# kakaoenterprise/JORLDY

Measured on AMD Instinct MI355X. Metric: env_steps_per_s (PPO CartPole sync, W=8 workers/GPU, T=128), higher is better.
Workload: dtype f32

## Files before the change

include/jorldy_hip.h:

```cpp
#ifndef JORLDY_HIP_H
#define JORLDY_HIP_H

#include <stdint.h>

#ifdef __cplusplus
extern "C" {
#endif

#define JH_ABI_VERSION 2

typedef enum {
  JH_OK = 0,
  JH_ERR_HIP = -1,
  JH_ERR_ARG = -2,
  JH_ERR_STATE = -3,
  JH_ERR_NOMEM = -4,
  JH_ERR_NODEVICE = -5
} jh_status;

typedef enum { JH_U8 = 0, JH_F32 = 1, JH_I64 = 2, JH_F64 = 3, JH_I32 = 4 } jh_dtype;

typedef struct jh_ctx jh_ctx;
typedef struct jh_store jh_store;
typedef struct jh_per jh_per;
// ... 37 lines not shown
void* jh_store_col_ptr(jh_store* s, int32_t col);
int64_t jh_store_size(const jh_store* s);
int64_t jh_store_index(const jh_store* s);
int64_t jh_store_capacity(const jh_store* s);
void jh_store_clear(jh_store* s);
int jh_store_set_position(jh_store* s, int64_t index, int64_t counter);

int jh_per_create(jh_ctx* ctx, int64_t capacity, double uniform_sample_prob, jh_per** out);
void jh_per_destroy(jh_per* p);
int jh_per_push(jh_per* p, int64_t n, const double* h_prio, jh_stream stream);
int jh_per_push_device(jh_per* p, int64_t n, const double* d_prio, jh_stream stream);
int jh_per_update(jh_per* p, int64_t B, const int64_t* d_idx, const void* d_prio, int32_t prio_dtype, jh_stream stream);
int jh_per_sample(jh_per* p, int64_t B, double beta, int64_t n_uniform, const int64_t* h_uniform_slot,
                  const double* h_u, int64_t* d_idx, double* d_w64, float* d_w32, double* d_stats, jh_stream stream);
int jh_per_shard_stats(jh_per* p, int64_t B, double* d_out3, jh_stream stream);
int jh_per_weights_sharded(jh_per* p, int64_t B, double beta, const double* d_all3, int32_t n_shards, double* d_w64,
                           float* d_w32, jh_stream stream);
int jh_per_state(jh_per* p, double* max_priority, double* root, int64_t* tree_index, int64_t* counter, jh_stream stream);
double* jh_per_tree_ptr(jh_per* p);
int64_t jh_per_tree_size(const jh_per* p);
int jh_per_load(jh_per* p, const double* h_tree, double max_priority, int64_t tree_index, int64_t counter);
int jh_per_dump(jh_per* p, double* h_tree, jh_stream stream);

int jh_gae(jh_ctx* ctx, int32_t W, int32_t T, float gamma, float lambda, const float* d_reward, const float* d_done,
           const float* d_value, const float* d_next_value, float* d_adv, float* d_ret, int32_t standardize,
           jh_stream stream);
int jh_ppo_minibatch_rows(jh_ctx* ctx, int64_t n, const int64_t* d_idx, int32_t n_cols, const int32_t* elems,
                          const float* const* d_src, float* const* d_dst, jh_stream stream);
int jh_mean_f32(jh_ctx* ctx, int64_t n, const float* d_x, float* d_out, jh_stream stream);
int jh_logp_discrete(jh_ctx* ctx, int64_t M, int32_t A, const float* d_logits, const float* d_action, float* d_logp,
                     jh_stream stream);
int jh_logp_continuous(jh_ctx* ctx, int64_t M, int32_t A, const float* d_mu_raw, const float* d_log_std_raw,
                       const float* d_action, float* d_logp, jh_stream stream);
int jh_ppo_loss_discrete(jh_ctx* ctx, int32_t B, int32_t A, const float* d_logits, const float* d_value_pred,
                         const int64_t* d_idx, const float* d_action, const float* d_adv, const float* d_ret,
                         const float* d_value_old, const float* d_logp_old, float eps_clip, float vf_coef,
                         float ent_coef, float* d_grad_logits, float* d_grad_value, float* d_stats,
                         jh_stream stream);
int jh_ppo_loss_continuous(jh_ctx* ctx, int32_t B, int32_t A, const float* d_mu_raw, const float* d_log_std_raw,
                           const float* d_value_pred, const int64_t* d_idx, const float* d_action, const float* d_adv,
                           const float* d_ret, const float* d_value_old, const float* d_logp_old, float eps_clip,
                           float vf_coef, float ent_coef, float* d_grad_mu_raw, float* d_grad_log_std_raw,
                           float* d_grad_value, float* d_stats, jh_stream stream);
int jh_ppo_loss_deferred(jh_ctx* ctx, int32_t continuous, int32_t B, int32_t A, const float* d_head0, const float* d_head1,
                         const float* d_value_pred, const int64_t* d_idx, const float* d_action, const float* d_adv, const float* d_ret,
                         const float* d_value_old, const float* d_logp_old, float eps_clip, float vf_coef, float ent_coef,
                         float* d_grad_head0, float* d_grad_head1, float* d_grad_value, float* d_dv2, float* d_critic_sums,
                         float* d_stats_local, jh_stream stream);
int jh_ppo_critic_select_rows(jh_ctx* ctx, int32_t B, const float* d_critic_sums, float vf_coef, float ent_coef, float* d_grad_value,
                              const float* d_dv2, const float* d_stats_local, float* d_stats, jh_stream stream);

int jh_ppo_loss_packed(jh_ctx* ctx, int32_t continuous, int32_t B, int32_t A, const float* d_heads, int32_t ld, const int64_t* d_idx, const float* d_action,
                       const float* d_adv, const float* d_ret, const float* d_value_old, const float* d_logp_old, float eps_clip, float vf_coef,
                       float ent_coef, float* d_grad_heads, float* d_dv2, float* d_critic_sums, float* d_stats, jh_stream stream);
int jh_ppo_critic_select_strided(jh_ctx* ctx, int32_t B, const float* d_critic_sums, float vf_coef, float ent_coef, float* d_grad_value, int32_t ldv,
                                 const float* d_dv2, const float* d_stats_local, float* d_stats, jh_stream stream);
int jh_heads_unpack(jh_ctx* ctx, int64_t rows, int32_t A, const float* d_packed, int32_t ld, float* d_h0, float* d_h1, float* d_value, jh_stream stream);
int jh_policy_act_discrete(jh_ctx* ctx, int32_t W, int32_t A, const float* d_heads, int32_t ld, uint64_t seed, uint64_t counter, int32_t training,
                           int64_t* d_action, jh_stream stream);

#define JH_TD_DOUBLE 1
#define JH_TD_PER 2
int jh_td_loss(jh_ctx* ctx, int32_t B, int32_t A, int32_t n_step, int32_t flags, const float* d_q,
               const float* d_q_next_online, const float* d_q_next_target, const float* d_action,
               const float* d_reward, const float* d_done, const float* d_weights, float gamma, float alpha,
               float* d_grad_q, float* d_prio, float* d_stats, jh_stream stream);
// ... 327 lines not shown
```

jorldy_amd/_lib.py:

```python
import ctypes as C
import os

_HERE = os.path.dirname(os.path.abspath(__file__))
LIB_PATH = os.path.join(_HERE, "csrc", "libjorldy_hip.so")

JH_U8, JH_F32, JH_I64, JH_F64, JH_I32 = 0, 1, 2, 3, 4
JH_TD_DOUBLE, JH_TD_PER = 1, 2
JH_C51_DOUBLE, JH_C51_PER, JH_C51_SHIFT_MAX = 1, 2, 4


class JhError(RuntimeError):
    pass


class ColDesc(C.Structure):
    _fields_ = [("dtype", C.c_int32), ("elems", C.c_int64)]


_vp, _i32, _i64, _f32, _f64 = C.c_void_p, C.c_int32, C.c_int64, C.c_float, C.c_double
_pp = C.POINTER(C.c_void_p)

_PROTOS = {
    "jh_abi_version": (C.c_int, []),
    "jh_stream_abort_capture": (C.c_int, [_vp]),
# ... 14 lines not shown
    "jh_pinned_free": (None, [_vp]),
    "jh_store_create": (C.c_int, [_vp, _i64, _i32, C.POINTER(ColDesc), _pp]),
    "jh_store_destroy": (None, [_vp]),
    "jh_store_push": (C.c_int, [_vp, _i64, _pp, _vp]),
    "jh_store_push_device": (C.c_int, [_vp, _i64, _pp, _vp]),
    "jh_store_stage_begin": (C.c_int, [_vp, _i64, _pp]),
    "jh_store_stage_commit": (C.c_int, [_vp, _vp]),
    "jh_store_write_rows": (C.c_int, [_vp, _i64, _vp, _pp, _vp]),
    "jh_store_gather": (C.c_int, [_vp, _i64, _vp, _i64, _i32, C.POINTER(_i32), _pp, C.POINTER(_i32), _vp]),
    "jh_store_col_ptr": (_vp, [_vp, _i32]),
    "jh_store_size": (_i64, [_vp]),
    "jh_store_index": (_i64, [_vp]),
    "jh_store_capacity": (_i64, [_vp]),
    "jh_store_clear": (None, [_vp]),
    "jh_store_set_position": (C.c_int, [_vp, _i64, _i64]),
    "jh_per_create": (C.c_int, [_vp, _i64, _f64, _pp]),
    "jh_per_destroy": (None, [_vp]),
    "jh_per_push": (C.c_int, [_vp, _i64, _vp, _vp]),
    "jh_per_push_device": (C.c_int, [_vp, _i64, _vp, _vp]),
    "jh_per_update": (C.c_int, [_vp, _i64, _vp, _vp, _i32, _vp]),
    "jh_per_sample": (C.c_int, [_vp, _i64, _f64, _i64, _vp, _vp, _vp, _vp, _vp, _vp, _vp]),
    "jh_per_state": (C.c_int, [_vp, C.POINTER(_f64), C.POINTER(_f64), C.POINTER(_i64), C.POINTER(_i64), _vp]),
    "jh_per_tree_ptr": (_vp, [_vp]),
    "jh_per_shard_stats": (C.c_int, [_vp, _i64, _vp, _vp]),
    "jh_per_weights_sharded": (C.c_int, [_vp, _i64, _f64, _vp, _i32, _vp, _vp, _vp]),
    "jh_per_tree_size": (_i64, [_vp]),
    "jh_per_load": (C.c_int, [_vp, _vp, _f64, _i64, _i64]),
    "jh_per_dump": (C.c_int, [_vp, _vp, _vp]),
    "jh_gae": (C.c_int, [_vp, _i32, _i32, _f32, _f32, _vp, _vp, _vp, _vp, _vp, _vp, _i32, _vp]),
    "jh_ppo_minibatch_rows": (C.c_int, [_vp, _i64, _vp, _i32, _vp, _vp, _vp, _vp]),
    "jh_mean_f32": (C.c_int, [_vp, _i64, _vp, _vp, _vp]),
    "jh_logp_discrete": (C.c_int, [_vp, _i64, _i32, _vp, _vp, _vp, _vp]),
    "jh_logp_continuous": (C.c_int, [_vp, _i64, _i32, _vp, _vp, _vp, _vp, _vp]),
    "jh_ppo_loss_discrete": (C.c_int, [_vp, _i32, _i32, _vp, _vp, _vp, _vp, _vp, _vp, _vp, _vp, _f32, _f32, _f32, _vp, _vp, _vp, _vp]),
    "jh_ppo_loss_continuous": (C.c_int, [_vp, _i32, _i32, _vp, _vp, _vp, _vp, _vp, _vp, _vp, _vp, _vp, _f32, _f32, _f32, _vp, _vp, _vp, _vp, _vp]),
    "jh_normal_fill": (C.c_int, [_vp, _i64, _vp, _vp, _vp]),
    "jh_value_act": (C.c_int, [_vp, _i32, _i32, _i32, _vp, _f32, _f32, _vp, _vp, _vp, _vp, _vp, _vp, _vp]),
    "jh_td_loss": (C.c_int, [_vp, _i32, _i32, _i32, _i32, _vp, _vp, _vp, _vp, _vp, _vp, _vp, _f32, _f32, _vp, _vp, _vp, _vp]),
    "jh_c51_loss": (C.c_int, [_vp, _i32, _i32, _i32, _i32, _i32, _vp, _vp, _vp, _vp, _vp, _vp, _vp, _f32, _f32, _f32, _f32, _vp, _vp, _vp, _vp, _vp]),
    "jh_mdqn_loss": (C.c_int, [_vp, _i32, _i32, _vp, _vp, _vp, _vp, _vp, _vp, _f32, _f32, _f32, _f32, _vp, _vp, _vp]),
    "jh_qr_loss": (C.c_int, [_vp, _i32, _i32, _i32, _vp, _vp, _vp, _vp, _vp, _vp, _vp, _f32, _vp, _vp, _vp]),
    "jh_quantile_act": (C.c_int, [_vp, _i32, _i32, _i32, _vp, _vp, _vp, _vp, _vp, _vp, _vp, _vp]),
    "jh_iqnnet_param_count_for": (_i64, [_i32, _i32, _i32, _i32, _i32]),
    "jh_iqnnet_create": (C.c_int, [_vp, _i32, _i32, _i32, _i32, _i32, _i32, _vp, _vp, _vp, _vp, _vp, _pp]),
    "jh_iqnnet_destroy": (None, [_vp]),
    "jh_iqnnet_segment_count": (_i32, []),
    "jh_iqnnet_segment": (C.c_int, [_vp, _i32, C.POINTER(_i64), C.POINTER(_i32), C.POINTER(_i32)]),
    "jh_iqnnet_set_hyper": (C.c_int, [_vp, _f64, _f64, _f64, _f64, _i64, _vp]),
    "jh_iqnnet_set_lr": (C.c_int, [_vp, _f64, _vp]),
    "jh_iqnnet_sync_target": (C.c_int, [_vp, _vp]),
    "jh_iqnnet_forward": (C.c_int, [_vp, _i32, _vp, _i32, _vp, _vp, _vp]),
    "jh_iqnnet_learn_forward": (C.c_int, [_vp, _vp, _i32, _vp, _vp, _vp]),
    "jh_iqnnet_learn_forward_m": (C.c_int, [_vp, _vp, _i32, _vp, _vp, _vp]),
    "jh_iqnnet_backward": (C.c_int, [_vp, _vp, _vp]),
    "jh_iqnnet_optim_step": (C.c_int, [_vp, _f32, _vp]),
    "jh_iqn_cos_features": (C.c_int, [_vp, _i64, _i32, _vp, _vp, _vp]),
    "jh_iqn_hadamard": (C.c_int, [_vp, _i32, _i32, _i32, _vp, _vp, _vp, _vp]),
    "jh_iqn_hadamard_backward": (C.c_int, [_vp, _i32, _i32, _i32, _vp, _vp, _vp, _vp, _vp, _vp]),
    "jh_iqn_loss": (C.c_int, [_vp, _i32, _i32, _i32, _vp, _vp, _vp, _vp, _vp, _vp, _vp, _f32, _vp, _vp, _vp]),
    "jh_miqn_loss": (C.c_int, [_vp, _i32, _i32, _i32, _vp, _vp, _vp, _vp, _vp, _vp, _vp, _f32, _f32, _f32, _f32, _vp, _vp, _vp]),
    "jh_iqn_act": (C.c_int, [_vp, _i32, _i32, _i32, _vp, _vp, _vp, _vp, _vp, _vp, _vp, _vp]),
    "jh_td3_next_action": (C.c_int, [_vp, _i32, _i32, _vp, _vp, _f32, _f32, _vp, _vp]),
    "jh_td3_critic_loss": (C.c_int, [_vp, _i32, _i32, _vp, _vp, _vp, _vp, _f32, _vp, _vp, _vp, _vp]),
    "jh_td3_actor_seed": (C.c_int, [_vp, _i32, _vp, _vp, _vp, _vp]),
    "jh_td3_tanh_backward": (C.c_int, [_vp, _i32, _i32, _vp, _vp, _vp, _vp]),
    "jh_td3_polyak": (C.c_int, [_vp, _i64, _vp, _vp, _f64, _vp]),
# ... 220 lines not shown
```

jorldy_amd/core/agent/ppo.py:

```python
import os

import numpy as np
import torch

from ... import np_rng, ops
from ..buffer import RolloutBuffer
from ..network import Network
from ..optimizer import Optimizer
from .base import BaseAgent


MAX_HEAD_OUTPUTS = 40
NATIVE_ELIGIBLE = ("PPO runs on libjorldy_hip only: network in {discrete_policy_value, continuous_policy_value}, head='mlp', int state_size, "
                   "hidden_size % 16 == 0, optim_config name 'adam' without weight_decay / amsgrad, and action_size + 1 (discrete) or "
                   f"2 * action_size + 1 (continuous) <= {MAX_HEAD_OUTPUTS} head outputs (config.ppo.cartpole, config.ppo.mujoco on all its envs; up to 8 outputs "
                   "-- CartPole, Hopper -- on the four-launch minibatch update and the persistent acting kernel, beyond that on the separate calls / the tiled engine); "
                   "head='cnn' with a (C, H, W) state_size and network 'discrete_policy_value' runs on the convolutional engine (core/agent/ppo_cnn.py: config.ppo.atari, ppo.procgen)")


class PPO(BaseAgent):

    def __new__(cls, *args, **kwargs):
        if cls is PPO and kwargs.get("head", args[4] if len(args) > 4 else "mlp") == "cnn":
            from .ppo_cnn import PPOConv

            return object.__new__(PPOConv)
        return object.__new__(cls)

    def __init__(self, state_size, action_size, hidden_size=512, network="discrete_policy_value", head="mlp",
                 optim_config={"name": "adam"}, gamma=0.99, use_standardization=True, run_step=1e6, lr_decay=True,
                 device=None, batch_size=32, n_step=128, n_epoch=3, _lambda=0.95, epsilon_clip=0.1, vf_coef=1.0,
                 ent_coef=0.01, clip_grad_norm=1.0, num_workers=1, backend=None, use_graph=True, seed=0, **kwargs):
        self.device = self._require_gpu(device)
        self.action_type = network.split("_")[0]
        assert self.action_type in ["continuous", "discrete"]
        if backend not in (None, "auto", "native"):
            raise ValueError(f"backend={backend!r}: jorldy_amd has one backend (libjorldy_hip); the torch mirror of round 1-3 is test infrastructure now (tests/mirror)")
        shape_ok = (head == "mlp" and isinstance(state_size, (int, np.integer)) and network in ("discrete_policy_value", "continuous_policy_value")
                    and hidden_size % 16 == 0 and optim_config.get("name", "adam").lower() == "adam"
                    and (2 * action_size + 1 if self.action_type == "continuous" else action_size + 1) <= MAX_HEAD_OUTPUTS)
        if not shape_ok:
            raise ValueError(f"{NATIVE_ELIGIBLE}; got network={network!r}, head={head!r}, state_size={state_size!r}, hidden_size={hidden_size}, "
                             f"optim_config={optim_config!r}, action_size={action_size}")
        self.network = Network(network, state_size, action_size, D_hidden=hidden_size, head=head).to(self.device)
        self.optimizer = Optimizer(**optim_config, params=self.network.parameters())
        self.gamma = gamma
        self.use_standardization = use_standardization
        self.memory = RolloutBuffer(device=self.device)
        self.run_step = run_step
        self.lr_decay = lr_decay
        self.batch_size = batch_size
        self.n_step = n_step
        self.n_epoch = n_epoch
# ... 2 lines not shown
        self.vf_coef = vf_coef
        self.ent_coef = ent_coef
        self.clip_grad_norm = clip_grad_norm
        self.num_workers = num_workers
        self.time_t = 0
        self.learn_stamp = 0
        self._stats = None
        self.grad_sync = None
        self.dp_exact_critic = os.environ.get("JH_DP_EXACT_CRITIC", "1") == "1"

        eligible = (
            head == "mlp" and isinstance(state_size, (int, np.integer)) and optim_config.get("name", "adam").lower() == "adam"
            and network in ("discrete_policy_value", "continuous_policy_value") and hidden_size % 16 == 0
            and not self.optimizer.defaults.get("amsgrad", False) and self.optimizer.defaults.get("weight_decay", 0) == 0
            and (2 * action_size + 1 if self.action_type == "continuous" else action_size + 1) <= MAX_HEAD_OUTPUTS
        )
        if not eligible:
            raise ValueError(f"{NATIVE_ELIGIBLE}; got network={network!r}, head={head!r}, state_size={state_size!r}, hidden_size={hidden_size}, "
                             f"optim_config={optim_config!r}, action_size={action_size}")
        self.backend = "native"
        self.use_graph = use_graph
        self.fused_update = os.environ.get("JH_FUSED_UPDATE", "1") == "1"
        self.graph_with_collective = os.environ.get("JH_GRAPH_DP", "1") == "1"
        self._net = None
        self._learn_graphs = ops.LearnGraphs("learn()")
        self._static = None
        self._adam_steps = 0
        self._captured = 0
        self._post_launch_hook = None
        self._lr_step = None
        self._ride, self._ride_done, self._ride_wait = None, False, {}
        self._lr_word = None
        self._predraw = np_rng.Predraw() if os.environ.get("JH_PPO_PREDRAW", "1") == "1" else None
        self._init_native(int(state_size), int(action_size), int(hidden_size), seed)

    def _init_native(self, S, A, H, seed, max_rows=4096):
        cont = self.action_type == "continuous"
        self._seed = seed
        net = ops.PPONet(S, H, A, cont, max_rows, self.device, seed=seed)
        params = list(self.network.parameters())
        assert sum(p.numel() for p in params) == net.n_params, "state_dict layout mismatch with libjorldy_hip"
        o = 0
        with torch.no_grad():
            for p in params:
                n = p.numel()
                net.params[o : o + n].copy_(p.reshape(-1))
                p.data = net.params[o : o + n].view_as(p)
                p.grad = net.grads[o : o + n].view_as(p)
                o += n
        self._views = [(p, net.m[a : a + p.numel()].view_as(p), net.v[a : a + p.numel()].view_as(p))
                       for p, a in zip(params, np.cumsum([0] + [q.numel() for q in params[:-1]]))]
        d = self.optimizer.defaults
        net.set_hyper(d["lr"], d["betas"][0], d["betas"][1], d["eps"], step=0.0)
        self._net = net

    def _grow_native(self, rows):
        if rows <= self._net.max_rows:
            return
        old = self._net
        S, H, A = old.S, old.H, old.A
        net = ops.PPONet(S, H, A, old.cont, max(rows, 2 * old.max_rows), self.device, seed=self._seed)
        for dst, src in ((net.params, old.params), (net.grads, old.grads), (net.m, old.m), (net.v, old.v)):
            dst.copy_(src)
        o = 0
        for p in self.network.parameters():
            n = p.numel()
# ... 75 lines not shown
            self._static = self._alloc_static(M)
            self.reset_graphs()
        st = self._static
        return st["h0"], st["h1"], st["value"], st["next_value"]

    def _drop_rides(self):
        if self._ride is not None:
            self._ride.clear_rides()
        self._ride_wait.clear()
        if self._static is not None:
            self._static["idx_ready"] = False

    def _upload_idx(self, st, draw, ride=False):
        k = st["idx_k"]
        st["idx_k"] = 1 - k
        if st["idx_ev"][k] is not None:
            st["idx_ev"][k].synchronize()
            st["idx_ev"][k] = None
        ok = draw(st["idx_pin"][k].np)
        if ok is False:
            return False
        if ride and self._ride is not None:
            self._ride.ride_along(0, st["idx_pin"][k].dev_ptr.value, st["idx"].data_ptr(), st["idx"].numel() * 8, keep=(st["idx_pin"][k], st["idx"]))
            self._ride_wait["idx"] = k
            return True
        self._ride_wait.pop("idx", None)
        st["idx"].copy_(st["idx_alias"][k])
        ev = torch.cuda.Event()
        ev.record()
        st["idx_ev"][k] = ev
        return True

    def _enqueue_learn(self, st, captured=False):
        self._enqueue_pre(st, captured)
        self._enqueue_main(st)

    def _enqueue_pre(self, st, captured=False):
        self._enqueue_gather(st)
        self._enqueue_pre_pass(st, captured)

    def _enqueue_gather(self, st):
        tr = st["tr"]
        self.memory._store.gather(st["arange"], as_float=True, out={k: tr[k] for k in tr})

    def _enqueue_pre_pass(self, st, captured=False):
        net, M = self._net, st["M"]
        cont = net.cont
        tr = st["tr"]
        if captured:
            pass
        elif 2 * M <= min(net.max_rows, 8192):
            net.forward(st["x_all"], out=(st["h0_all"], st["h1_all"], st["v_all"]))
        else:
            net.forward(tr["next_state"], out=(st["nh0"], st["nh1"], st["next_value"]))
            net.forward(tr["state"], out=(st["h0"], st["h1"], st["value"]))
        if cont:
            logp_old = ops.logp_continuous(st["h0"], st["h1"], tr["action"], out=st["logp_old"])
        else:
            logp_old = ops.logp_discrete(st["h0"], tr["action"], out=st["logp_old"])
        adv, ret = ops.gae(tr["reward"], tr["done"], st["value"], st["next_value"], self.n_step, self.gamma, self._lambda, self.use_standardization,
                           out=(st["adv"], st["ret"]))
        ops.mean_into(ret, st["stats"][st["n_upd"], 0:1])

    def _enqueue_main(self, st):
        net, M, B = self._net, st["M"], self.batch_size
        cont = net.cont
        tr, adv, ret, logp_old = st["tr"], st["adv"], st["ret"], st["logp_old"]
        k = 0
        if "rows" in st:
            xs, acts, advs, rets, vals, lps = st["rows"](st["idx"])
            exact = self.grad_sync is not None and self.dp_exact_critic
            if exact and "critic_sums" not in st:
                st["critic_sums"] = torch.zeros(st["n_upd"], 2, dtype=torch.float32, device=self.device)
            for e in range(self.n_epoch):
                for offset in range(0, M, B):
                    o0, o1 = e * M + offset, e * M + min(offset + B, M)
                    if exact:
                        net.ppo_update_dp(xs[o0:o1], None, acts[o0:o1], advs[o0:o1], rets[o0:o1], vals[o0:o1], lps[o0:o1], self.epsilon_clip, self.vf_coef,
                                          self.ent_coef, st["stats"][k], self.grad_sync.reduce_flat, st["critic_sums"][k],
                                          peer=getattr(getattr(self.grad_sync, "transport", None), "peer", None))
                    else:
                        net.ppo_update(xs[o0:o1], None, acts[o0:o1], advs[o0:o1], rets[o0:o1], vals[o0:o1], lps[o0:o1], self.epsilon_clip, self.vf_coef,
                                       self.ent_coef, self.clip_grad_norm, st["stats"][k], do_adam=self.grad_sync is None)
                    if self.grad_sync is not None:
                        self.grad_sync.reduce_flat(net.grads)
                        net.adam_step(self.clip_grad_norm)
                    k += 1
            return
        exact = self.grad_sync is not None and self.dp_exact_critic
        if exact and "dp_work" not in st:
            st["dp_work"] = torch.zeros(st["n_upd"], B + 16, dtype=torch.float32, device=self.device)
        onepass = not exact and os.environ.get("JH_PPO_ONEPASS", "1") == "1"
        for e in range(self.n_epoch):
            for offset in range(0, M, B):
                b = min(B, M - offset)
                idx = st["idx"][e * M + offset : e * M + offset + b]
                if onepass:
                    net.ppo_update_rows(tr["state"], idx, tr["action"], adv, ret, st["value"], logp_old, self.epsilon_clip, self.vf_coef, self.ent_coef, self.clip_grad_norm,
                                        st["stats"][k], do_adam=self.grad_sync is None)
                    if self.grad_sync is not None:
                        self.grad_sync.reduce_flat(net.grads)
                        net.adam_step(self.clip_grad_norm)
                    k += 1
# ... 45 lines not shown
        self._captured = 0
        rode, self._ride_done = self._ride_done, False
        if self._ride_wait and not rode:
            if "lr" in self._ride_wait:
                self._net.set_lr(float(self._lr_word.np[0]))
            if "idx" in self._ride_wait and st["idx_ready"]:
                st["idx"].copy_(st["idx_alias"][self._ride_wait["idx"]])
        self._ride_wait.clear()

        def shuffles():
            self._upload_idx(st, lambda out: np_rng.epoch_shuffles(M, E, out))

        pin = st.get("stats_pin")
        if pin is not None:
            pin.np[st["n_upd"] - 1, 2] = -1.0
            pin.np[st["n_upd"] - 1, 7] = -1.0
        graphable = (self.use_graph and not ops._PROF["on"]
                     and (self.grad_sync is None or (self.graph_with_collective and getattr(self.grad_sync, "capturable", True))))
        have_idx = bool(st["idx_ready"]) and self._predraw is not None and self._predraw.commit(M, E)
        st["idx_ready"] = False
        split = not have_idx and os.environ.get("JH_PPO_SPLIT_GRAPH", "1") == "1"
        key = ("split" if split else "one", captured)
        lg, pre = self._learn_graphs, lambda: self._enqueue_pre(st, captured)
        bodies = {key: pre, "main": lambda: self._enqueue_main(st)} if split else {key: lambda: self._enqueue_learn(st, captured)}
        if lg.ready(key, bodies, graphable, warm_key=key, capture=allow_capture):
            if split:
                lg.replay(key)
                shuffles()
                lg.replay("main")
            else:
                if not have_idx:
                    shuffles()
                lg.replay(key)
        else:
            pre()
            if not have_idx:
                shuffles()
            self._enqueue_main(st)
            lg.warm.add(key)
        self.memory._store.clear()
        self._adam_steps += st["n_upd"]
        self._launched = (st, pin, M, E)

    def _learn_finish(self):
        st, pin, M, E = self._launched
        self._launched = None
        if self._lr_step is not None:
            if self.lr_decay:
                self.learning_rate_decay(self._lr_step)
            self._lr_step = None
        if self._predraw is not None:
            st["idx_ready"] = bool(self._upload_idx(st, lambda out: self._predraw.draw(M, E, out), ride=True))
        hook, self._post_launch_hook = self._post_launch_hook, None
        if hook is not None:
            hook()
        if pin is not None:
            s = self._await_mapped_stats(pin.np, st["n_upd"])
        else:
            s = self._read_stats(st["stats"])[0].astype(np.float64)
        return self._result(s, st["n_upd"])

    def _await_mapped_stats(self, a, n_upd):
        self._await_marks(a, ((n_upd - 1) * 8 + 2, (n_upd - 1) * 8 + 7), "PPO.learn()")
        return a.astype(np.float64)

    def learning_rate_decay(self, step, optimizers=None, mode="cosine"):
        super().learning_rate_decay(step, optimizers, mode)
        if self._net is not None:
            lr = self.optimizer.param_groups[0]["lr"]
            if self._ride is not None and self._lr_step is not None:
                if self._lr_word is None:
                    self._lr_word = ops.PinnedBuffer((1,), np.float32, self.device.index)
# ... 87 lines not shown
```

jorldy_amd/csrc/jh_ppo.hip:

```cpp
#include "jh_common.h"
#include "jh_peer.h"
#include "jh_ppo_finish.h"

__global__ void __launch_bounds__(256) jh_gae_kernel(int W, int T, float gamma, float lambda,
                                                     const float* __restrict__ reward,
                                                     const float* __restrict__ done,
                                                     const float* __restrict__ value,
                                                     const float* __restrict__ next_value,
                                                     float* __restrict__ adv, float* __restrict__ ret,
                                                     int standardize) {
  const int lane = threadIdx.x & 63;
  const int row = blockIdx.x * 4 + (threadIdx.x >> 6);
  if (row >= W) return;
  const size_t base = (size_t)row * (size_t)T;
  const int ntiles = (T + 63) >> 6;
  float carry = 0.f;
  float sum = 0.f;
  for (int k = ntiles - 1; k >= 0; --k) {
    const int t = k * 64 + lane;
    float a = 1.f, b = 0.f, v = 0.f;
    if (t < T) {
      const float r = reward[base + t], d = done[base + t], vn = next_value[base + t];
      v = value[base + t];
      const float nd_g = (1.f - d) * gamma;
      b = r + nd_g * vn - v;
      a = (t == T - 1) ? 0.f : nd_g * lambda;
    }
#pragma unroll
    for (int off = 1; off < 64; off <<= 1) {
      const float a2 = __shfl_down(a, off, 64);
      const float b2 = __shfl_down(b, off, 64);
      if (lane + off < 64) {
        b = b + a * b2;
        a = a * a2;
      }
    }
    const float x = b + a * carry;
    carry = __shfl(x, 0, 64);
    if (t < T) {
      adv[base + t] = x;
      ret[base + t] = x + v;
      sum += x;
    }
  }
  if (!standardize) return;
  const float mean = jh_wave_sum(sum) / (float)T;
  float ssq = 0.f;
  for (int t = lane; t < T; t += 64) {
    const float c = adv[base + t] - mean;
    ssq += c * c;
  }
  const float var = jh_wave_sum(ssq) / (float)(T - 1);
  const float inv = 1.f / (sqrtf(var) + 1e-7f);
  for (int t = lane; t < T; t += 64) adv[base + t] = (adv[base + t] - mean) * inv;
}

template <int E>
__global__ void __launch_bounds__(1024) jh_gae_long_kernel(int T, int nw, float gamma, float lambda, const float* __restrict__ reward,
                                                           const float* __restrict__ done, const float* __restrict__ value,
                                                           const float* __restrict__ next_value, float* __restrict__ adv, float* __restrict__ ret,
                                                           int standardize) {
  __shared__ float s_A[16 * E], s_B[16 * E], s_carry[16 * E + 1];
  __shared__ float s_red[16];
  const int lane = threadIdx.x & 63, wid = threadIdx.x >> 6;
  const size_t base = (size_t)blockIdx.x * (size_t)T;
  const int ntiles = (T + 63) >> 6;
  float a[E], b[E], v[E];
#pragma unroll
  for (int e = 0; e < E; ++e) {
    const int k = wid + nw * e, t = k * 64 + lane;
    a[e] = 1.f; b[e] = 0.f; v[e] = 0.f;
    if (k < ntiles && t < T) {
      const float r = reward[base + t], d = done[base + t], vn = next_value[base + t];
      v[e] = value[base + t];
      const float nd_g = (1.f - d) * gamma;
      b[e] = r + nd_g * vn - v[e];
      a[e] = (t == T - 1) ? 0.f : nd_g * lambda;
    }
  }
#pragma unroll
  for (int e = 0; e < E; ++e) {
#pragma unroll
    for (int off = 1; off < 64; off <<= 1) {
      const float a2 = __shfl_down(a[e], off, 64);
      const float b2 = __shfl_down(b[e], off, 64);
      if (lane + off < 64) {
        b[e] = b[e] + a[e] * b2;
// ... 195 lines not shown
  float z[kDiscCache];
  float m, lse, s;
  float p[kDiscCache], pn[kDiscCache], c[kDiscCache], lg[kDiscCache];
  bool inr[kDiscCache];
};

__device__ __forceinline__ void disc_reg_prepare(DiscReg& t, int A) {
  float m = t.z[0];
#pragma unroll
  for (int k = 1; k < kDiscCache; ++k)
    if (k < A) m = fmaxf(m, t.z[k]);
  float se = 0.f;
#pragma unroll
  for (int k = 0; k < kDiscCache; ++k)
    if (k < A) se += expf(t.z[k] - m);
  t.m = m;
  t.lse = logf(se);
  float s = 0.f;
#pragma unroll
  for (int k = 0; k < kDiscCache; ++k) {
    t.p[k] = 0.f;
    if (k < A) { t.p[k] = expf((t.z[k] - m) - t.lse); s += t.p[k]; }
  }
  t.s = s;
#pragma unroll
  for (int k = 0; k < kDiscCache; ++k) {
    t.pn[k] = t.p[k] / s;
    t.inr[k] = (t.pn[k] >= JH_EPS32) && (t.pn[k] <= 1.f - JH_EPS32);
    t.c[k] = fminf(fmaxf(t.pn[k], JH_EPS32), 1.f - JH_EPS32);
    t.lg[k] = logf(t.c[k]);
  }
}

__global__ void __launch_bounds__(256) jh_logp_discrete_kernel(int64_t M, int A, const float* __restrict__ logits,
                                                               const float* __restrict__ action,
                                                               float* __restrict__ logp) {
  const int64_t i = (int64_t)blockIdx.x * 256 + threadIdx.x;
  if (i >= M) return;
  const float* z = logits + i * A;
  float m = z[0];
  for (int k = 1; k < A; ++k) m = fmaxf(m, z[k]);
  float se = 0.f;
  for (int k = 0; k < A; ++k) se += expf(z[k] - m);
  int a = (int)action[i];
  a = a < 0 ? 0 : (a >= A ? A - 1 : a);
  const float pi = expf((z[a] - m) - logf(se));
  logp[i] = logf(pi);
}

__device__ __forceinline__ NormalD normal_terms(float mu_raw, float ls_raw, float act) {
  NormalD n;
  n.mu = fmin(fmax((double)mu_raw, -5.0), 5.0);
  n.th = tanh((double)ls_raw);
  n.std = exp(n.th);
  const float a = fminf(fmaxf(act, JH_ATANH_LO), JH_ATANH_HI);
  n.z = atanh((double)a);
  const double dm = n.z - n.mu;
  n.lp = -(dm * dm) / (2.0 * n.std * n.std) - log(n.std) - 0.91893853320467274178;
  return n;
}
__device__ __forceinline__ float normal_logp(float mu_raw, float ls_raw, float act, float& mu, float& std, float& z) {
  const NormalD n = normal_terms(mu_raw, ls_raw, act);
  mu = (float)n.mu; std = (float)n.std; z = (float)n.z;
  return (float)n.lp;
}

__global__ void __launch_bounds__(256) jh_logp_continuous_kernel(int64_t MA, const float* __restrict__ mu_raw,
                                                                 const float* __restrict__ ls_raw,
                                                                 const float* __restrict__ action,
                                                                 float* __restrict__ logp) {
  const int64_t i = (int64_t)blockIdx.x * 256 + threadIdx.x;
  if (i >= MA) return;
  float mu, std, z;
  logp[i] = normal_logp(mu_raw[i], ls_raw[i], action[i], mu, std, z);
}

JH_EXPORT int jh_logp_discrete(jh_ctx* ctx, int64_t M, int32_t A, const float* d_logits, const float* d_action,
                               float* d_logp, jh_stream stream) {
  JH_ARG(ctx && d_logits && d_action && d_logp);
  JH_ARG(M > 0 && A > 0);
  JH_LAUNCH(jh_logp_discrete_kernel, dim3((unsigned)((M + 255) / 256)), dim3(256), 0, jh_s(stream), M, A,
                     d_logits, d_action, d_logp);
  JH_LAUNCH_CHECK();
  return JH_OK;
}

JH_EXPORT int jh_logp_continuous(jh_ctx* ctx, int64_t M, int32_t A, const float* d_mu_raw, const float* d_log_std_raw,
                                 const float* d_action, float* d_logp, jh_stream stream) {
  JH_ARG(ctx && d_mu_raw && d_log_std_raw && d_action && d_logp);
  JH_ARG(M > 0 && A > 0);
  const int64_t MA = M * A;
  JH_LAUNCH(jh_logp_continuous_kernel, dim3((unsigned)((MA + 255) / 256)), dim3(256), 0, jh_s(stream), MA,
                     d_mu_raw, d_log_std_raw, d_action, d_logp);
  JH_LAUNCH_CHECK();
  return JH_OK;
}

struct RowCommon {
  float ratio, adv, v, vold, ret, vclip, smin;
  float g1, g2;
  bool in_clip, in_v;
};

__device__ __forceinline__ RowCommon row_common(float logp_diff_sum, float adv, float v, float vold, float ret,
                                                float eps) {
  RowCommon c;
  c.ratio = expf(logp_diff_sum);
  c.adv = adv;
  c.v = v;
  c.vold = vold;
  c.ret = ret;
  const float surr1 = c.ratio * adv;
  const float rc = fminf(fmaxf(c.ratio, 1.f - eps), 1.f + eps);
  const float surr2 = rc * adv;
  c.smin = fminf(surr1, surr2);
  c.g1 = surr1 < surr2 ? 1.f : (surr1 == surr2 ? 0.5f : 0.f);
  c.g2 = surr2 < surr1 ? 1.f : (surr1 == surr2 ? 0.5f : 0.f);
  c.in_clip = (c.ratio >= 1.f - eps) && (c.ratio <= 1.f + eps);
  const float dv = v - vold;
  c.in_v = (dv >= -eps) && (dv <= eps);
  c.vclip = vold + fminf(fmaxf(dv, -eps), eps);
  return c;
}


template <bool CONT>
// ... 786 lines not shown
```

jorldy_amd/ops.py:

```python
import contextlib
import ctypes as C

import numpy as np
import torch

from . import _lib as L

_DT = {torch.uint8: L.JH_U8, torch.float32: L.JH_F32, torch.int64: L.JH_I64, torch.float64: L.JH_F64, torch.int32: L.JH_I32, torch.bool: L.JH_U8}
_NP_DT = {np.dtype("uint8"): L.JH_U8, np.dtype("float32"): L.JH_F32, np.dtype("int64"): L.JH_I64, np.dtype("float64"): L.JH_F64, np.dtype("int32"): L.JH_I32, np.dtype("bool"): L.JH_U8}
_TORCH_OF = {L.JH_U8: torch.uint8, L.JH_F32: torch.float32, L.JH_I64: torch.int64, L.JH_F64: torch.float64, L.JH_I32: torch.int32}
_NP_OF = {L.JH_U8: np.uint8, L.JH_F32: np.float32, L.JH_I64: np.int64, L.JH_F64: np.float64, L.JH_I32: np.int32}


_PROF = {"on": False, "ev": {}, "lib": False}


class _timed:
    def __init__(self, name, nbytes, bound="hbm"):
        self.name, self.nbytes, self.bound = name, nbytes, bound

    def __enter__(self):
        if _PROF["on"]:
            self.e0 = torch.cuda.Event(enable_timing=True)
            self.e0.record()
# ... 339 lines not shown
        ret = torch.empty(M, dtype=torch.float32, device=r.device)
    else:
        adv, ret = (_f32(t).reshape(-1) for t in out)
    with _timed("jh_gae_kernel", 24 * M):
      L.check(lib.jh_gae(L.ctx(_dev(r)), M // n_step, int(n_step), float(gamma), float(lam), L.ptr(r), L.ptr(d), L.ptr(v), L.ptr(vn), L.ptr(adv), L.ptr(ret), int(bool(standardize)), L.stream_ptr()))
    return adv.view(-1, 1), ret.view(-1, 1)


def mean_into(x, out):
    x = _f32(x).reshape(-1)
    L.check(L.load().jh_mean_f32(L.ctx(_dev(x)), int(x.numel()), L.ptr(x), L.ptr(out), L.stream_ptr()))
    return out


class MinibatchRows:

    def __init__(self, srcs, dsts):
        self.lib = L.load()
        assert len(srcs) == len(dsts) <= 8
        self.srcs, self.dsts = [_f32(t) for t in srcs], list(dsts)
        n = len(srcs)
        self.n = int(dsts[0].shape[0])
        el = [int(t.numel() // t.shape[0]) for t in self.srcs]
        assert all(int(d.numel()) == self.n * e and d.is_contiguous() for d, e in zip(self.dsts, el))
        self._elems = (C.c_int32 * n)(*el)
        self._src = (C.c_void_p * n)(*[t.data_ptr() for t in self.srcs])
        self._dst = (C.c_void_p * n)(*[t.data_ptr() for t in self.dsts])
        self.ctx = L.ctx(_dev(self.srcs[0]))

    def __call__(self, idx):
        assert idx.dtype == torch.int64 and int(idx.numel()) == self.n
        L.check(self.lib.jh_ppo_minibatch_rows(self.ctx, self.n, L.ptr(idx), len(self.srcs), self._elems, self._src, self._dst, L.stream_ptr()))
        return self.dsts


def logp_discrete(logits, action, out=None):
    lib = L.load()
    z = _f32(logits)
    M, A = z.shape
    a = _f32(action).reshape(-1)
    out = torch.empty(M, dtype=torch.float32, device=z.device) if out is None else _f32(out).reshape(-1)
    L.check(lib.jh_logp_discrete(L.ctx(_dev(z)), M, A, L.ptr(z), L.ptr(a), L.ptr(out), L.stream_ptr()))
    return out.view(-1, 1)


def logp_continuous(mu_raw, log_std_raw, action, out=None):
    lib = L.load()
    mu, ls, a = _f32(mu_raw), _f32(log_std_raw), _f32(action)
    M, A = mu.shape
    out = torch.empty(M, A, dtype=torch.float32, device=mu.device) if out is None else _f32(out)
    L.check(lib.jh_logp_continuous(L.ctx(_dev(mu)), M, A, L.ptr(mu), L.ptr(ls), L.ptr(a), L.ptr(out), L.stream_ptr()))
    return out


def ppo_loss_discrete(logits, value_pred, idx, action, adv, ret, value_old, logp_old, eps_clip, vf_coef, ent_coef, stats=None):
    lib = L.load()
    z, v = _f32(logits), _f32(value_pred).reshape(-1)
    B, A = z.shape
    g_z = torch.empty_like(z)
    g_v = torch.empty(B, dtype=torch.float32, device=z.device)
    if stats is None:
        stats = torch.empty(8, dtype=torch.float32, device=z.device)
    with _timed("jh_ppo_fused_kernel" if B <= 1024 else "jh_ppo_fwd+bwd", 4 * B * (2 * A + 7) + 8 * B):
      L.check(lib.jh_ppo_loss_discrete(L.ctx(_dev(z)), B, A, L.ptr(z), L.ptr(v), L.ptr(idx), L.ptr(_f32(action).reshape(-1)), L.ptr(_f32(adv).reshape(-1)), L.ptr(_f32(ret).reshape(-1)), L.ptr(_f32(value_old).reshape(-1)), L.ptr(_f32(logp_old).reshape(-1)), float(eps_clip), float(vf_coef), float(ent_coef), L.ptr(g_z), L.ptr(g_v), L.ptr(stats), L.stream_ptr()))
    return g_z, g_v.view(-1, 1), stats

# ... 1409 lines not shown
```

Measured before the change: 1.217 million.

## Fuse PPO pre-update stages into a single prologue kernel

Result: no change. 1.219 million, median of 2 (+0.2%).

```diff
diff --git a/include/jorldy_hip.h b/include/jorldy_hip.h
--- a/include/jorldy_hip.h
+++ b/include/jorldy_hip.h
@@ -93,6 +93,10 @@
                      jh_stream stream);
 int jh_logp_continuous(jh_ctx* ctx, int64_t M, int32_t A, const float* d_mu_raw, const float* d_log_std_raw,
                        const float* d_action, float* d_logp, jh_stream stream);
+int jh_ppo_prologue(jh_ctx* ctx, jh_store* s, const int32_t* cols, int32_t A, int32_t continuous, const float* d_h0,
+                    const float* d_h1, const float* d_value, const float* d_next_value, float* const* d_tr, float* d_logp_old,
+                    float* d_adv, float* d_ret, float* d_mean, float* const* d_mb, const int64_t* d_idx, int32_t E, int32_t W,
+                    int32_t T, float gamma, float lambda, int32_t standardize, jh_stream stream);
 int jh_ppo_loss_discrete(jh_ctx* ctx, int32_t B, int32_t A, const float* d_logits, const float* d_value_pred,
                          const int64_t* d_idx, const float* d_action, const float* d_adv, const float* d_ret,
                          const float* d_value_old, const float* d_logp_old, float eps_clip, float vf_coef,
diff --git a/jorldy_amd/_lib.py b/jorldy_amd/_lib.py
--- a/jorldy_amd/_lib.py
+++ b/jorldy_amd/_lib.py
@@ -70,6 +70,7 @@
     "jh_mean_f32": (C.c_int, [_vp, _i64, _vp, _vp, _vp]),
     "jh_logp_discrete": (C.c_int, [_vp, _i64, _i32, _vp, _vp, _vp, _vp]),
     "jh_logp_continuous": (C.c_int, [_vp, _i64, _i32, _vp, _vp, _vp, _vp, _vp]),
+    "jh_ppo_prologue": (C.c_int, [_vp, _vp, _vp, _i32, _i32, _vp, _vp, _vp, _vp, _vp, _vp, _vp, _vp, _vp, _vp, _vp, _i32, _i32, _i32, _f32, _f32, _i32, _vp]),
     "jh_ppo_loss_discrete": (C.c_int, [_vp, _i32, _i32, _vp, _vp, _vp, _vp, _vp, _vp, _vp, _vp, _f32, _f32, _f32, _vp, _vp, _vp, _vp]),
     "jh_ppo_loss_continuous": (C.c_int, [_vp, _i32, _i32, _vp, _vp, _vp, _vp, _vp, _vp, _vp, _vp, _vp, _f32, _f32, _f32, _vp, _vp, _vp, _vp, _vp]),
     "jh_normal_fill": (C.c_int, [_vp, _i64, _vp, _vp, _vp]),
diff --git a/jorldy_amd/core/agent/ppo.py b/jorldy_amd/core/agent/ppo.py
--- a/jorldy_amd/core/agent/ppo.py
+++ b/jorldy_amd/core/agent/ppo.py
@@ -18,7 +18,29 @@
                    "head='cnn' with a (C, H, W) state_size and network 'discrete_policy_value' runs on the convolutional engine (core/agent/ppo_cnn.py: config.ppo.atari, ppo.procgen)")
 
 
+PROLOGUE_HOOKS = ("_enqueue_pre", "_enqueue_pre_pass", "_enqueue_gather", "_enqueue_main")
+
+
+def prologue_switch():
+    return os.environ.get("JH_PPO_PROLOGUE", "1") == "1"
+
+
+def prologue_eligible(cls, switch, captured, has_rows, form, M, T, S, A, cont, columns, capacity):
+    if not (switch and captured and has_rows and form == "one"):
+        return False
+    if not all(getattr(cls, h) is getattr(PPO, h) for h in PROLOGUE_HOOKS):
+        return False
+    if M % T != 0 or not ops.ppo_prologue_fits(M, T, S, A, cont):
+        return False
+    cols = {c[0]: int(c[2]) for c in (columns or ())}
+    want = {"state": S, "action": A if cont else 1, "reward": 1, "next_state": S, "done": 1}
+    return all(cols.get(k) == v for k, v in want.items()) and M <= capacity
+
+
 class PPO(BaseAgent):
+
+    use_prologue = False
+    last_pre_path = None
 
     def __new__(cls, *args, **kwargs):
         if cls is PPO and kwargs.get("head", args[4] if len(args) > 4 else "mlp") == "cnn":
@@ -87,6 +109,8 @@
         self._ride, self._ride_done, self._ride_wait = None, False, {}
         self._lr_word = None
         self._predraw = np_rng.Predraw() if os.environ.get("JH_PPO_PREDRAW", "1") == "1" else None
+        self.use_prologue = prologue_switch()
+        self.last_pre_path = None
         self._init_native(int(state_size), int(action_size), int(hidden_size), seed)
 
     def _init_native(self, S, A, H, seed, max_rows=4096):
@@ -228,8 +252,32 @@
         return True
 
     def _enqueue_learn(self, st, captured=False):
+        paths = self.__dict__.setdefault("_pre_paths", {})
+        paths["one", captured] = "five"
+        if self._prologue_ok(st, captured):
+            paths["one", captured] = "prologue"
+            self._enqueue_prologue(st)
+            self._enqueue_main(st, rows_done=True)
+            return
         self._enqueue_pre(st, captured)
         self._enqueue_main(st)
+
+    def _prologue_ok(self, st, captured, form="one"):
+        if not (self.use_prologue and captured and "rows" in st):
+            return False
+        store = self.memory._store
+        return prologue_eligible(type(self), self.use_prologue, captured, "rows" in st, form, st["M"], self.n_step, self._net.S, self._net.A, self._net.cont,
+                                 None if store is None else store.columns, 0 if store is None else store.capacity)
+
+    def _enqueue_prologue(self, st):
+        store = self.memory._store
+        pro = st.get("prologue")
+        if pro is None or pro.store is not store:
+            M = st["M"]
+            pro = st["prologue"] = ops.PPOPrologue(store, st["tr"], st["h0"], st["h1"], st["value"], st["next_value"], st["logp_old"], st["adv"], st["ret"],
+                                                   st["stats"][st["n_upd"], 0:1], st["mb"], st["idx"], self.n_epoch, M // self.n_step, self.n_step,
+                                                   self.gamma, self._lambda, self.use_standardization)
+        pro()
 
     def _enqueue_pre(self, st, captured=False):
         self._enqueue_gather(st)
@@ -258,13 +306,13 @@
                            out=(st["adv"], st["ret"]))
         ops.mean_into(ret, st["stats"][st["n_upd"], 0:1])
 
-    def _enqueue_main(self, st):
+    def _enqueue_main(self, st, rows_done=False):
         net, M, B = self._net, st["M"], self.batch_size
         cont = net.cont
         tr, adv, ret, logp_old = st["tr"], st["adv"], st["ret"], st["logp_old"]
         k = 0
         if "rows" in st:
-            xs, acts, advs, rets, vals, lps = st["rows"](st["idx"])
+            xs, acts, advs, rets, vals, lps = st["mb"] if rows_done else st["rows"](st["idx"])
             exact = self.grad_sync is not None and self.dp_exact_critic
             if exact and "critic_sums" not in st:
                 st["critic_sums"] = torch.zeros(st["n_upd"], 2, dtype=torch.float32, device=self.device)
@@ -376,12 +424,16 @@
                 if not have_idx:
                     shuffles()
                 lg.replay(key)
+        elif have_idx:
+            self._enqueue_learn(st, captured)
+            lg.warm.add(key)
         else:
             pre()
-            if not have_idx:
-                shuffles()
+            shuffles()
             self._enqueue_main(st)
             lg.warm.add(key)
+            self.__dict__.get("_pre_paths", {}).pop(key, None)
+        self.last_pre_path = self.__dict__.get("_pre_paths", {}).get(key, "five")
         self.memory._store.clear()
         self._adam_steps += st["n_upd"]
         self._launched = (st, pin, M, E)
diff --git a/jorldy_amd/csrc/jh_ppo.hip b/jorldy_amd/csrc/jh_ppo.hip
--- a/jorldy_amd/csrc/jh_ppo.hip
+++ b/jorldy_amd/csrc/jh_ppo.hip
@@ -1,6 +1,37 @@
 #include "jh_common.h"
 #include "jh_peer.h"
 #include "jh_ppo_finish.h"
+
+__device__ __forceinline__ void gae_terms(float r, float d, float vn, float v, bool row_end, float gamma, float lambda, float& a, float& b) {
+  const float nd_g = (1.f - d) * gamma;
+  b = r + nd_g * vn - v;
+  a = row_end ? 0.f : nd_g * lambda;
+}
+__device__ __forceinline__ float gae_tile_scan(float a, float b, int lane, float& carry) {
+#pragma unroll
+  for (int off = 1; off < 64; off <<= 1) {
+    const float a2 = __shfl_down(a, off, 64);
+    const float b2 = __shfl_down(b, off, 64);
+    if (lane + off < 64) {
+      b = b + a * b2;
+      a = a * a2;
+    }
+  }
+  const float x = b + a * carry;
+  carry = __shfl(x, 0, 64);
+  return x;
+}
+__device__ __forceinline__ void gae_standardize_row(float* adv_row, int T, int lane, float sum) {
+  const float mean = jh_wave_sum(sum) / (float)T;
+  float ssq = 0.f;
+  for (int t = lane; t < T; t += 64) {
+    const float c = adv_row[t] - mean;
+    ssq += c * c;
+  }
+  const float var = jh_wave_sum(ssq) / (float)(T - 1);
+  const float inv = 1.f / (sqrtf(var) + 1e-7f);
+  for (int t = lane; t < T; t += 64) adv_row[t] = (adv_row[t] - mean) * inv;
+}
 
 __global__ void __launch_bounds__(256) jh_gae_kernel(int W, int T, float gamma, float lambda,
                                                      const float* __restrict__ reward,
@@ -22,21 +53,9 @@
     if (t < T) {
       const float r = reward[base + t], d = done[base + t], vn = next_value[base + t];
       v = value[base + t];
-      const float nd_g = (1.f - d) * gamma;
-      b = r + nd_g * vn - v;
-      a = (t == T - 1) ? 0.f : nd_g * lambda;
-    }
-#pragma unroll
-    for (int off = 1; off < 64; off <<= 1) {
-      const float a2 = __shfl_down(a, off, 64);
-      const float b2 = __shfl_down(b, off, 64);
-      if (lane + off < 64) {
-        b = b + a * b2;
-        a = a * a2;
-      }
-    }
-    const float x = b + a * carry;
-    carry = __shfl(x, 0, 64);
+      gae_terms(r, d, vn, v, t == T - 1, gamma, lambda, a, b);
+    }
+    const float x = gae_tile_scan(a, b, lane, carry);
     if (t < T) {
       adv[base + t] = x;
       ret[base + t] = x + v;
@@ -44,15 +63,7 @@
     }
   }
   if (!standardize) return;
-  const float mean = jh_wave_sum(sum) / (float)T;
-  float ssq = 0.f;
-  for (int t = lane; t < T; t += 64) {
-    const float c = adv[base + t] - mean;
-    ssq += c * c;
-  }
-  const float var = jh_wave_sum(ssq) / (float)(T - 1);
-  const float inv = 1.f / (sqrtf(var) + 1e-7f);
-  for (int t = lane; t < T; t += 64) adv[base + t] = (adv[base + t] - mean) * inv;
+  gae_standardize_row(adv + base, T, lane, sum);
 }
 
 template <int E>
@@ -314,20 +325,23 @@
   }
 }
 
+__device__ __forceinline__ float logp_discrete_row(const float* __restrict__ z, int A, float action) {
+  float m = z[0];
+  for (int k = 1; k < A; ++k) m = fmaxf(m, z[k]);
+  float se = 0.f;
+  for (int k = 0; k < A; ++k) se += expf(z[k] - m);
+  int a = (int)action;
+  a = a < 0 ? 0 : (a >= A ? A - 1 : a);
+  const float pi = expf((z[a] - m) - logf(se));
+  return logf(pi);
+}
+
 __global__ void __launch_bounds__(256) jh_logp_discrete_kernel(int64_t M, int A, const float* __restrict__ logits,
                                                                const float* __restrict__ action,
                                                                float* __restrict__ logp) {
   const int64_t i = (int64_t)blockIdx.x * 256 + threadIdx.x;
   if (i >= M) return;
-  const float* z = logits + i * A;
-  float m = z[0];
-  for (int k = 1; k < A; ++k) m = fmaxf(m, z[k]);
-  float se = 0.f;
-  for (int k = 0; k < A; ++k) se += expf(z[k] - m);
-  int a = (int)action[i];
-  a = a < 0 ? 0 : (a >= A ? A - 1 : a);
-  const float pi = expf((z[a] - m) - logf(se));
-  logp[i] = logf(pi);
+  logp[i] = logp_discrete_row(logits + i * A, A, action[i]);
 }
 
 __device__ __forceinline__ NormalD normal_terms(float mu_raw, float ls_raw, float act) {
@@ -374,6 +388,252 @@
   const int64_t MA = M * A;
   JH_LAUNCH(jh_logp_continuous_kernel, dim3((unsigned)((MA + 255) / 256)), dim3(256), 0, jh_s(stream), MA,
                      d_mu_raw, d_log_std_raw, d_action, d_logp);
+  JH_LAUNCH_CHECK();
+  return JH_OK;
+}
+
+#ifndef JH_PPO_PROLOGUE_ROWS
+#define JH_PPO_PROLOGUE_ROWS 256
+#endif
+constexpr int kPrologueRows = JH_PPO_PROLOGUE_ROWS;
+constexpr int kPrologueMaxS = 16;
+constexpr int kPrologueMaxLds = 65536;
+struct PrologueArgs {
+  int M, W, T, E, S, A, aw, lw;
+  int rows_per_wg;
+  int vec4;
+  float gamma, lambda;
+  int standardize;
+  const void* col[5];
+  int dt[5];
+  const float *h0, *h1, *value, *next_value;
+  float* tr[5];
+  float *logp_old, *adv, *ret, *mean;
+  float* mb[6];
+  const int64_t* idx;
+};
+
+__device__ __forceinline__ float prologue_col(const void* p, int dt, int64_t i) {
+  switch (dt) {
+    case JH_U8: return (float)((const uint8_t*)p)[i];
+    case JH_I64: return (float)((const int64_t*)p)[i];
+    case JH_F64: return (float)((const double*)p)[i];
+    case JH_I32: return (float)((const int32_t*)p)[i];
+    default: return ((const float*)p)[i];
+  }
+}
+
+template <bool STD, bool CONT, int C>
+__device__ __forceinline__ float prologue_at(const PrologueArgs& a, int64_t i) {
+  if (!STD) return prologue_col(a.col[C], a.dt[C], i);
+  if (C == 4) return (float)((const uint8_t*)a.col[C])[i];
+  if (C == 1 && !CONT) return (float)((const int64_t*)a.col[C])[i];
+  return ((const float*)a.col[C])[i];
+}
+
+struct PrologueGaeIn {
+  float r[4], d[4], vn[4], v[4];
+};
+template <bool STD, bool CONT>
+__device__ __forceinline__ PrologueGaeIn prologue_gae_load(const PrologueArgs& a, int row, int lane) {
+  PrologueGaeIn in;
+  const int64_t base = (int64_t)row * a.T;
+#pragma unroll
+  for (int k = 0; k < 4; ++k) {
+    const int t = k * 64 + lane;
+    in.r[k] = 0.f; in.d[k] = 0.f; in.vn[k] = 0.f; in.v[k] = 0.f;
+    if (t < a.T) {
+      in.r[k] = prologue_at<STD, CONT, 2>(a, base + t);
+      in.d[k] = prologue_at<STD, CONT, 4>(a, base + t);
+      in.vn[k] = a.next_value[base + t];
+      in.v[k] = a.value[base + t];
+    }
+  }
+  return in;
+}
+
+template <bool CONT>
+struct PrologueRow {
+  int64_t r;
+  float s[kPrologueMaxS];
+  float act[CONT ? kContCache : 1];
+  float val;
+};
+template <bool STD, bool CONT>
+__device__ __forceinline__ void prologue_row_fetch(const PrologueArgs& a, PrologueRow<CONT>& p) {
+  if (a.vec4) {
+    const float4* src = reinterpret_cast<const float4*>(a.col[0]) + p.r * (a.S >> 2);
+#pragma unroll
+    for (int q = 0; q < kPrologueMaxS / 4; ++q) {
+      const float4 v = 4 * q < a.S ? src[q] : make_float4(0.f, 0.f, 0.f, 0.f);
+      p.s[4 * q] = v.x; p.s[4 * q + 1] = v.y; p.s[4 * q + 2] = v.z; p.s[4 * q + 3] = v.w;
+    }
+  } else {
+#pragma unroll
+    for (int k = 0; k < kPrologueMaxS; ++k) p.s[k] = k < a.S ? prologue_at<STD, CONT, 0>(a, p.r * a.S + k) : 0.f;
+  }
+#pragma unroll
+  for (int k = 0; k < (CONT ? kContCache : 1); ++k) p.act[k] = k < a.aw ? prologue_at<STD, CONT, 1>(a, p.r * a.aw + k) : 0.f;
+  p.val = a.value[p.r];
+}
+
+template <bool STD, bool CONT, int C>
+__device__ __forceinline__ void prologue_copy(const PrologueArgs& a, int64_t tot, int64_t gt, int64_t gs) {
+  if ((C == 0 || C == 3) && a.vec4) {
+    for (int64_t j = gt; j < (tot >> 2); j += gs) reinterpret_cast<float4*>(a.tr[C])[j] = reinterpret_cast<const float4*>(a.col[C])[j];
+  } else {
+    for (int64_t j = gt; j < tot; j += gs) a.tr[C][j] = prologue_at<STD, CONT, C>(a, j);
+  }
+}
+
+template <bool CONT, bool STD>
+__global__ void __launch_bounds__(1024) jh_ppo_prologue_kernel(PrologueArgs a) {
+  extern __shared__ float s_dyn[];
+  float* s_adv = s_dyn;
+  float* s_ret = s_dyn + a.M;
+  float* s_logp = s_dyn + 2 * (size_t)a.M;
+  const int tid = threadIdx.x, lane = tid & 63, wid = tid >> 6;
+  const int M = a.M;
+  const int64_t n = (int64_t)a.E * M;
+  const int64_t g0 = (int64_t)blockIdx.x * a.rows_per_wg;
+  const int64_t g1 = g0 + a.rows_per_wg < n ? g0 + a.rows_per_wg : n;
+
+  int64_t i = g0 + tid;
+  PrologueRow<CONT> p;
+  p.r = 0;
+  if (i < g1) {
+    const int64_t r = a.idx[i];
+    p.r = r < 0 ? 0 : (r >= M ? M - 1 : r);
+  }
+  int row = wid;
+  PrologueGaeIn in{};
+  if (row < a.W) in = prologue_gae_load<STD, CONT>(a, row, lane);
+
+  if (CONT) {
+    for (int j = tid; j < M * a.A; j += 1024) {
+      float mu, std, z;
+      s_logp[j] = normal_logp(a.h0[j], a.h1[j], prologue_at<STD, CONT, 1>(a, j), mu, std, z);
+    }
+  } else {
+    for (int m = tid; m < M; m += 1024) s_logp[m] = logp_discrete_row(a.h0 + (size_t)m * a.A, a.A, prologue_at<STD, CONT, 1>(a, m));
+  }
+  if (i < g1) prologue_row_fetch<STD, CONT>(a, p);
+
+  const int ntiles = (a.T + 63) >> 6;
+  while (row < a.W) {
+    const int base = row * a.T;
+    float carry = 0.f, sum = 0.f;
+#pragma unroll
+    for (int k = 3; k >= 0; --k) {
+      if (k < ntiles) {
+        const int t = k * 64 + lane;
+        float ga = 1.f, gb = 0.f, v = 0.f;
+        if (t < a.T) {
+          v = in.v[k];
+          gae_terms(in.r[k], in.d[k], in.vn[k], v, t == a.T - 1, a.gamma, a.lambda, ga, gb);
+        }
+        const float x = gae_tile_scan(ga, gb, lane, carry);
+        if (t < a.T) {
+          s_adv[base + t] = x;
+          s_ret[base + t] = x + v;
+          sum += x;
+        }
+      }
+    }
+    row += 16;
+    if (row < a.W) in = prologue_gae_load<STD, CONT>(a, row, lane);
+    if (a.standardize) gae_standardize_row(s_adv + base, a.T, lane, sum);
+  }
+  __syncthreads();
+
+  while (i < g1) {
+    if (a.vec4) {
+      float4* dst = reinterpret_cast<float4*>(a.mb[0]) + i * (a.S >> 2);
+#pragma unroll
+      for (int q = 0; q < kPrologueMaxS / 4; ++q)
+        if (4 * q < a.S) dst[q] = make_float4(p.s[4 * q], p.s[4 * q + 1], p.s[4 * q + 2], p.s[4 * q + 3]);
+    } else {
+#pragma unroll
+      for (int k = 0; k < kPrologueMaxS; ++k)
+        if (k < a.S) a.mb[0][i * a.S + k] = p.s[k];
+    }
+#pragma unroll
+    for (int k = 0; k < (CONT ? kContCache : 1); ++k)
+      if (k < a.aw) a.mb[1][i * a.aw + k] = p.act[k];
+    if (CONT)
+      for (int k = kContCache; k < a.aw; ++k) a.mb[1][i * a.aw + k] = prologue_at<STD, CONT, 1>(a, p.r * a.aw + k);
+    a.mb[2][i] = s_adv[p.r];
+    a.mb[3][i] = s_ret[p.r];
+    a.mb[4][i] = p.val;
+    for (int k = 0; k < a.lw; ++k) a.mb[5][i * a.lw + k] = s_logp[p.r * a.lw + k];
+    i += 1024;
+    if (i < g1) {
+      const int64_t r = a.idx[i];
+      p.r = r < 0 ? 0 : (r >= M ? M - 1 : r);
+      prologue_row_fetch<STD, CONT>(a, p);
+    }
+  }
+
+  if (blockIdx.x == 0) {
+    for (int m = tid; m < M; m += 1024) { a.adv[m] = s_adv[m]; a.ret[m] = s_ret[m]; }
+    for (int j = tid; j < M * a.lw; j += 1024) a.logp_old[j] = s_logp[j];
+    float acc = 0.f;
+    for (int m = tid; m < M; m += 1024) acc += s_ret[m];
+    acc = jh_block_reduce(acc, s_dyn, JhAdd(), 0.f);
+    if (tid == 0) *a.mean = acc / (float)(int64_t)M;
+  }
+
+  const int64_t gt = (int64_t)blockIdx.x * 1024 + tid, gs = (int64_t)gridDim.x * 1024;
+  prologue_copy<STD, CONT, 0>(a, (int64_t)M * a.S, gt, gs);
+  prologue_copy<STD, CONT, 1>(a, (int64_t)M * a.aw, gt, gs);
+  prologue_copy<STD, CONT, 2>(a, M, gt, gs);
+  prologue_copy<STD, CONT, 3>(a, (int64_t)M * a.S, gt, gs);
+  prologue_copy<STD, CONT, 4>(a, M, gt, gs);
+}
+
+JH_EXPORT int jh_ppo_prologue(jh_ctx* ctx, jh_store* s, const int32_t* cols, int32_t A, int32_t continuous, const float* d_h0, const float* d_h1,
+                              const float* d_value, const float* d_next_value, float* const* d_tr, float* d_logp_old, float* d_adv, float* d_ret,
+                              float* d_mean, float* const* d_mb, const int64_t* d_idx, int32_t E, int32_t W, int32_t T, float gamma, float lambda,
+                              int32_t standardize, jh_stream stream) {
+  JH_ARG(ctx && s && cols && d_h0 && d_value && d_next_value && d_tr && d_logp_old && d_adv && d_ret && d_mean && d_mb && d_idx);
+  JH_ARG(!continuous || d_h1);
+  JH_ARG(E > 0 && W > 0 && T > 0 && T <= 256 && A > 0);
+  JH_ARG((int64_t)W * T <= s->capacity && (int64_t)W * T * E < (int64_t)1 << 30);
+  PrologueArgs a{};
+  a.M = W * T; a.W = W; a.T = T; a.E = E; a.A = A;
+  a.aw = a.lw = continuous ? A : 1;
+  for (int c = 0; c < 5; ++c) {
+    JH_ARG(cols[c] >= 0 && cols[c] < s->n_cols && d_tr[c]);
+    a.col[c] = s->dev[cols[c]]; a.dt[c] = s->cols[cols[c]].dtype; a.tr[c] = d_tr[c];
+  }
+  const int64_t S = s->cols[cols[0]].elems;
+  JH_ARG(S > 0 && S <= kPrologueMaxS && s->cols[cols[3]].elems == S);
+  JH_ARG(s->cols[cols[1]].elems == a.aw && s->cols[cols[2]].elems == 1 && s->cols[cols[4]].elems == 1);
+  a.S = (int)S;
+  a.vec4 = S % 4 == 0 && a.dt[0] == JH_F32 && a.dt[3] == JH_F32
+           && (((uintptr_t)a.col[0] | (uintptr_t)a.col[3] | (uintptr_t)d_tr[0] | (uintptr_t)d_tr[3] | (uintptr_t)d_mb[0]) & 15) == 0;
+  const size_t lds = (size_t)(2 + a.lw) * 4 * (size_t)a.M;
+  if (lds > (size_t)kPrologueMaxLds)
+    return jh_fail(JH_ERR_ARG, "jh_ppo_prologue: %d rows need %zu bytes of LDS per workgroup (limit %d): use the separate launches", a.M, lds, kPrologueMaxLds);
+  for (int c = 0; c < 6; ++c) {
+    JH_ARG(d_mb[c] != nullptr);
+    a.mb[c] = d_mb[c];
+  }
+  a.gamma = gamma; a.lambda = lambda; a.standardize = standardize;
+  a.h0 = d_h0; a.h1 = d_h1; a.value = d_value; a.next_value = d_next_value;
+  a.logp_old = d_logp_old; a.adv = d_adv; a.ret = d_ret; a.mean = d_mean; a.idx = d_idx;
+  const int64_t n = (int64_t)E * a.M;
+  int64_t g = (n + kPrologueRows - 1) / kPrologueRows;
+  a.rows_per_wg = kPrologueRows;
+  if (g > 256) { g = 256; a.rows_per_wg = (int)((n + g - 1) / g); }
+  const bool std_types = a.dt[0] == JH_F32 && a.dt[2] == JH_F32 && a.dt[3] == JH_F32 && a.dt[4] == JH_U8 && a.dt[1] == (continuous ? JH_F32 : JH_I64);
+#define JH_PROLOGUE(CONT, STD) \
+  JH_LAUNCH_NAMED("jh_ppo_prologue", (jh_ppo_prologue_kernel<CONT, STD>), dim3((unsigned)g), dim3(1024), lds < 64 ? 64 : lds, jh_s(stream), a)
+  if (continuous && std_types) JH_PROLOGUE(true, true);
+  else if (continuous) JH_PROLOGUE(true, false);
+  else if (std_types) JH_PROLOGUE(false, true);
+  else JH_PROLOGUE(false, false);
+#undef JH_PROLOGUE
   JH_LAUNCH_CHECK();
   return JH_OK;
 }
diff --git a/jorldy_amd/ops.py b/jorldy_amd/ops.py
--- a/jorldy_amd/ops.py
+++ b/jorldy_amd/ops.py
@@ -395,6 +395,39 @@
         assert idx.dtype == torch.int64 and int(idx.numel()) == self.n
         L.check(self.lib.jh_ppo_minibatch_rows(self.ctx, self.n, L.ptr(idx), len(self.srcs), self._elems, self._src, self._dst, L.stream_ptr()))
         return self.dsts
+
+
+PROLOGUE_MAX_T, PROLOGUE_MAX_S, PROLOGUE_MAX_LDS = 256, 16, 65536
+
+
+def ppo_prologue_fits(M, T, S, A, continuous):
+    return 0 < T <= PROLOGUE_MAX_T and 0 < S <= PROLOGUE_MAX_S and (2 + (A if continuous else 1)) * 4 * M <= PROLOGUE_MAX_LDS
+
+
+class PPOPrologue:
+
+    NAMES = ("state", "action", "reward", "next_state", "done")
+
+    def __init__(self, store, tr, h0, h1, value, next_value, logp_old, adv, ret, mean_out, mb, idx, E, W, T, gamma, lam, standardize):
+        self.lib = L.load()
+        M = W * T
+        A = int(h0.shape[1])
+        self.store = store
+        self._cols = (C.c_int32 * 5)(*[store.names.index(nm) for nm in self.NAMES])
+        self._keep = [h0, value, next_value, logp_old, adv, ret, mean_out] + [tr[nm] for nm in self.NAMES] + list(mb) + ([] if h1 is None else [h1])
+        assert all(t.dtype == torch.float32 and t.is_cuda and t.is_contiguous() for t in self._keep), "static float32 CUDA buffers"
+        assert int(h0.numel()) == M * A and int(value.numel()) == M == int(next_value.numel()) == int(adv.numel()) == int(ret.numel())
+        assert idx.dtype == torch.int64 and idx.is_contiguous() and int(idx.numel()) == E * M and len(mb) == 6 and all(int(t.shape[0]) == E * M for t in mb)
+        self._tr = (C.c_void_p * 5)(*[tr[nm].data_ptr() for nm in self.NAMES])
+        self._mb = (C.c_void_p * 6)(*[t.data_ptr() for t in mb])
+        self.h1, self.idx, self.mb = h1, idx, list(mb)
+        self.ctx = L.ctx(_dev(h0))
+        self._args = (A, int(h1 is not None), L.ptr(h0), L.ptr(h1), L.ptr(value), L.ptr(next_value), self._tr, L.ptr(logp_old), L.ptr(adv), L.ptr(ret),
+                      L.ptr(mean_out), self._mb, L.ptr(idx), int(E), int(W), int(T), float(gamma), float(lam), int(bool(standardize)))
+
+    def __call__(self):
+        L.check(self.lib.jh_ppo_prologue(self.ctx, self.store.h, self._cols, *self._args, L.stream_ptr()))
+        return self.mb
 
 
 def logp_discrete(logits, action, out=None):
```
